# Nico59000/Ternary-image-codec

Measured on AMD Instinct MI355X. Metric: Mpix/s encode+decode 8K RS(26,20), higher is better.
Workload: dtype u8

## Files before the change

### ternary-image-codec_amd/csrc/t3_api.cpp

```cpp
#include <hip/hip_runtime.h>
#include <math.h>
#include <stdio.h>
#include <stdlib.h>
#include <string.h>

#include <algorithm>
#include <atomic>
#include <map>
#include <mutex>
#include <string>
#include <system_error>
#include <thread>
#include <tuple>
#include <vector>

#include "../../include/t3hip.h"
#include "t3_ctx.hpp"
#include "t3_host.hpp"
#include "t3_kernels.h"
#include "t3_decode.h"

using namespace t3;

namespace {
// ... 252 lines not shown
      fprintf(stderr, "[t3 stamps]   CUs seen=%zu  CUs holding n WGs: 1:%d 2:%d 3:%d 4:%d 5:%d 6+:%d\n", per_cu.size(), hist[1], hist[2], hist[3], hist[4], hist[5], hist[6] + hist[7]);
      fprintf(stderr, "[t3 stamps]   mean WG lifetime (us) per XCC:"); for (int x = 0; x < 8; ++x) fprintf(stderr, " %d:%.1f(n=%d)", x, xn[x] ? xl[x] / xn[x] : 0.0, xn[x]); fprintf(stderr, "\n");
      double ln[8] = {0}; int cn[8] = {0}; for (auto& kv : per_cu) { const size_t n = std::min<size_t>(kv.second.size(), 7); for (uint32_t v : kv.second) { ln[n] += v * 0.01; ++cn[n]; } }
      fprintf(stderr, "[t3 stamps]   mean WG lifetime (us) by WGs on its CU:"); for (int n = 1; n < 8; ++n) if (cn[n]) fprintf(stderr, " %d:%.1f", n, ln[n] / cn[n]); fprintf(stderr, "\n");
      fprintf(stderr, "[t3 stamps]   hw_id samples: %08x %08x %08x %08x\n", (unsigned)h16[8], (unsigned)h16[16 + 8], (unsigned)h16[32 + 8], (unsigned)h16[16 * 100 + 8]); }
    double acc[8] = {0, 0, 0, 0, 0, 0, 0, 0};
    for (uint32_t w = 0; w < grid; ++w) for (int i = 0; i < 8; ++i) acc[i] += (double)h[8 * w + i];
    fprintf(stderr, "[t3 stamps] grid=%u tiles=%u  mean cycles/WG: stage=%.0f p1=%.0f p2=%.0f p3=%.0f total=%.0f  clock=%.3f GHz\n", grid, e.a.n_tiles,
            acc[0] / grid, acc[1] / grid, acc[2] / grid, acc[3] / grid, acc[4] / grid, acc[4] / acc[5] * 0.1);
    { uint64_t s0 = ~0ull, s1 = 0, e0 = ~0ull, e1 = 0; for (uint32_t w = 0; w < grid; ++w) { const uint64_t st = h[8 * w + 3], en = st + h[8 * w + 5]; s0 = std::min(s0, st); s1 = std::max(s1, st); e0 = std::min(e0, en); e1 = std::max(e1, en); }
      int late = 0; for (uint32_t w = 0; w < grid; ++w) if (h[8 * w + 3] - s0 > 1000) ++late;
      fprintf(stderr, "[t3 stamps]   timeline (us from first start): last start=%.2f first end=%.2f last end=%.2f  WGs starting >10us late=%d\n", (s1 - s0) * 0.01, (e0 - s0) * 0.01, (e1 - s0) * 0.01, late);
      fprintf(stderr, "[t3 stamps]   lds_bytes=%u block=%u\n", e.a.lds_bytes, e.block); }
    fprintf(stderr, "[t3 stamps]   p1 split (wave 0): prefetch issue=%.0f convert=%.0f barrier wait=%.0f\n", acc[6] / grid, acc[7] / grid, acc[1] / grid);
    { double il = 0; for (uint32_t w = 0; w < grid; ++w) il += (double)h16[16 * w + 10]; fprintf(stderr, "[t3 stamps]   2-D permutation pass (in p2): %.0f\n", il / grid); }
    return T3_OK;
}
#endif

int launch_enc(Ctx& c, EncLaunch& e, hipStream_t s) {
    uint32_t grid; { const int rc = resident_grid(c, e.fn, (int)e.block, e.a.lds_bytes, e.a.n_tiles, true, &grid); if (rc) return rc; }
#ifdef T3_STAMPS
    static uint64_t* d_dbg = nullptr; static int calls = 0;
    if (!d_dbg) HIPCHK(hipMalloc((void**)&d_dbg, 16 * 8 * 4096));
    HIPCHK(hipMemsetAsync(d_dbg, 0, 16 * 8 * 4096, s));
    e.a.dbg = d_dbg;
#endif
    tile_tickets_held(c, s, 0, grid, &e.a.tile_ctr, &e.a.n_classes);
    void* args[] = {(void*)&e.a};
    HIPCHK(hipLaunchKernel(e.fn, dim3(grid), dim3(e.block), args, e.a.lds_bytes, s));
// ... 360 lines not shown
    t3_layout L; int rc = plan(n_raw, *cfg, L); if (rc) return rc;
    *n_out = L.out_words; if (L.out_words > cap) return T3_E_CAPACITY;
    std::lock_guard<std::recursive_mutex> hl(c.host_mu);
    void *di, *dout;
    { std::lock_guard<std::mutex> lk(c.mu); rc = scratch_held(c, Scratch::HostIn, n_units * (fe == FE_PIXELS ? 6 : 9) + 64, &di); if (rc) return rc; rc = scratch_held(c, Scratch::HostOut, L.out_words * 9 + 64, &dout); if (rc) return rc; }
    rc = encode_host_pipelined(c, fe, in, n_units, cfg, out, L, di, dout);
    if (rc != 1) return rc;
    if (n_units) HIPCHK(hipMemcpyAsync(di, in, n_units * (fe == FE_PIXELS ? 6 : 9), hipMemcpyHostToDevice, c.stream));
    rc = encode_dev(fe, di, n_units, cfg, dout, L.out_words, n_out, c.stream); if (rc) return rc;
    if (L.out_words) HIPCHK(hipMemcpyAsync(out, dout, L.out_words * 9, hipMemcpyDeviceToHost, c.stream));
    HIPCHK(hipStreamSynchronize(c.stream)); return T3_OK;
}
int t3hip_encode_profile(const void* raw, uint64_t n_raw, const t3_cfg* cfg, void* out, uint64_t cap, uint64_t* n_out) { return encode_host(FE_WORDS, raw, n_raw, cfg, out, cap, n_out); }
int t3hip_encode_frame(const void* px, uint64_t n_px, const t3_cfg* cfg, void* out, uint64_t cap, uint64_t* n_out) { return encode_host(FE_PIXELS, px, n_px, cfg, out, cap, n_out); }

int t3hip_event_create(void** ev) { if (!ctx().ready) return T3_E_NODEVICE; hipEvent_t e; HIPCHK(hipEventCreate(&e)); *ev = e; return T3_OK; }
int t3hip_event_record(void* ev, void* stream) { HIPCHK(hipEventRecord((hipEvent_t)ev, (hipStream_t)stream)); return T3_OK; }
int t3hip_event_elapsed_ms(void* a, void* b, float* ms) { HIPCHK(hipEventSynchronize((hipEvent_t)b)); HIPCHK(hipEventElapsedTime(ms, (hipEvent_t)a, (hipEvent_t)b)); return T3_OK; }
int t3hip_event_destroy(void* ev) { HIPCHK(hipEventDestroy((hipEvent_t)ev)); return T3_OK; }

}

namespace t3 {
int encode_rgb_fused(const void* d_rgb, uint64_t n_px, const t3_cfg* cfg, void* d_out, uint64_t cap, uint64_t* n_out, hipStream_t s) { return encode_dev(FE_RGB, d_rgb, n_px, cfg, d_out, cap, n_out, s); }
int scratch(Ctx& c, Scratch kind, size_t bytes, void** out, hipStream_t s) { std::lock_guard<std::mutex> lk(c.mu); return scratch_held(c, kind, bytes, out, s); }
void tile_tickets(Ctx& c, hipStream_t s, int kind, uint32_t grid, uint32_t** ctr, uint32_t* n_classes) { std::lock_guard<std::mutex> lk(c.mu); tile_tickets_held(c, s, kind, grid, ctr, n_classes); }
int resident_grid(Ctx& c, const void* fn, int threads, uint32_t lds_bytes, uint64_t n_items, bool round_lds_units, uint32_t* grid) {
    static std::map<std::tuple<const void*, int, int, uint32_t>, int> occ; static std::mutex occ_mu;
    int per_cu;
    {
        std::lock_guard<std::mutex> lk(occ_mu);
// ... 70 lines not shown
```

### ternary-image-codec_amd/csrc/t3_api_decode.cpp

```cpp
#include <hip/hip_runtime.h>
#include <math.h>
#include <stdio.h>
#include <string.h>

#include <stdlib.h>

#include <algorithm>
#include <mutex>
#include <vector>

#include "../../include/t3hip.h"
#include "t3_ctx.hpp"
#include "t3_decode.h"
#include "t3_host.hpp"
#include "t3_window.h"

using namespace t3;

namespace {
struct HdrCheck { HdrExpect ex; uint32_t hs; uint32_t* verdict; const uint8_t* in; };

int launch_hdr_compare(const HdrCheck* h, hipStream_t s) {
    if (!h) return T3_OK;
    hipLaunchKernelGGL(hdr_compare_kernel, dim3(1), dim3(128), 0, s, h->in, h->ex, h->hs, h->verdict);
// ... 152 lines not shown
    void* args[] = {(void*)&a};
    HIPCHK(hipLaunchKernel(p.fn, dim3(grid), dim3(p.threads), args, a.lds_bytes, s));
#ifdef T3_DEC_STAMPS
    if (++calls == 8 && p.tickets) {
        std::vector<uint64_t> h(16 * grid);
        HIPCHK(hipStreamSynchronize(s));
        HIPCHK(hipMemcpy(h.data(), d_dbg, h.size() * 8, hipMemcpyDeviceToHost));
        double acc[16] = {0};
        for (uint32_t w = 0; w < grid; ++w) for (int i = 0; i < 16; ++i) acc[i] += (double)h[16 * w + i];
        fprintf(stderr, "[t3 dec stamps] grid=%u (%d per CU) tiles=%u lds=%u  mean cycles/WG: producer sets+e1=%.0f barrier=%.0f total=%.0f | consumer bm=%.0f rendezvous=%.0f d5=%.0f barrier=%.0f total=%.0f  clock=%.3f GHz  us/WG=%.1f\n",
                grid, (int)((grid + c.n_cu - 1) / c.n_cu), a.n_tiles, a.lds_bytes, acc[0] / grid, acc[1] / grid, acc[6] / grid, acc[8 + 2] / grid, acc[8 + 3] / grid, acc[8 + 4] / grid, acc[8 + 5] / grid, acc[8 + 6] / grid,
                acc[6] / acc[7] * 0.1, acc[7] / grid * 0.01);
        uint64_t s0 = ~0ull, s1 = 0, e1 = 0; int late = 0;
        for (uint32_t w = 0; w < grid; ++w) { s0 = std::min(s0, h[16 * w + 2]); s1 = std::max(s1, h[16 * w + 2]); e1 = std::max(e1, h[16 * w + 3]); }
        for (uint32_t w = 0; w < grid; ++w) if (h[16 * w + 2] - s0 > 1000) ++late;
        fprintf(stderr, "[t3 dec stamps]   timeline (us from first loop start): last start=%.1f last end=%.1f  workgroups starting >10 us late=%d\n", (s1 - s0) * 0.01, (e1 - s0) * 0.01, late);
    }
#endif
    return T3_OK;
}

struct UepPlan { DecUepArgs a; const void* fn; uint32_t grid; };
int plan_fixed_uep(uint64_t body_bytes, uint32_t hdr_syms, const t3_cfg& cfg, const t3_layout& L, const ScrCycle& sc,
                   void* d_out, uint64_t units, uint32_t* d_fail, UepPlan& p) {
    if (L.n_raw_words == 0 || L.n_sym + (1u << 20) >= (1ull << 32) || body_bytes + hdr_syms >= (1ull << 32)) return 1;
    if (getenv("T3HIP_TWO_KERNEL_DECODE") != nullptr) return 1;
    if (body_bytes >= (1ull << 28)) return 1;
    const bool il = L.interleave2d != 0 && cfg.tile_w > 1;
    DecUepArgs& a = p.a; memset(&a, 0, sizeof a);
    int gk[kUepMaxGrp]; uint32_t gn[kUepMaxGrp];
// ... 462 lines not shown
```

### ternary-image-codec_amd/csrc/t3_api_record.cpp

```cpp
#include <hip/hip_runtime.h>
#include <stdlib.h>
#include <string.h>

#include <algorithm>
#include <mutex>
#include <vector>

#include "../../include/t3hip.h"
#include "t3_crc.h"
#include "t3_ctx.hpp"

using namespace t3;

namespace {
struct CrcOp {
    uint32_t col[32];
    uint32_t apply(uint32_t v) const { uint32_t r = 0; for (int b = 0; b < 32; ++b) if (v >> b & 1u) r ^= col[b]; return r; }
    static CrcOp compose(const CrcOp& a, const CrcOp& b) { CrcOp r; for (int i = 0; i < 32; ++i) r.col[i] = a.apply(b.col[i]); return r; }
    static CrcOp identity() { CrcOp r; for (int b = 0; b < 32; ++b) r.col[b] = 1u << b; return r; }
    static CrcOp zero_byte() {
        CrcOp r;
        for (int b = 0; b < 32; ++b) { uint32_t v = 1u << b; for (int i = 0; i < 8; ++i) v = (v & 1u) ? (0xEDB88320u ^ (v >> 1)) : (v >> 1); r.col[b] = v; }
        return r;
    }
// ... 51 lines not shown
    if (mfma) {
        CrcMArgs& m = p.m;
        m.data = d_data; m.n_bytes = n_bytes; m.n_rounds = (uint32_t)(n_bytes >> 11);
        const uint32_t slots = crc_slots(c);
        m.rounds_per_wave = (uint32_t)std::max<uint64_t>(8, ((uint64_t)m.n_rounds + slots - 1) / slots);
        m.afrag = c.crc.afrag4; m.zpow = c.crc.zpow; m.chunk_crc = acc; m.sym_sum = acc + 1;
        m.tail_len = (uint32_t)(n_bytes - ((uint64_t)m.n_rounds << 11));
        const uint32_t tail_wg = m.tail_len ? 1u : 0u;
        if (knob.blocked) {
            const uint64_t waves = ((uint64_t)m.n_rounds + m.rounds_per_wave - 1) / m.rounds_per_wave;
            p.form = CrcForm::Fp4Blocked; p.m_grid = (uint32_t)((waves + 3) / 4 + tail_wg);
        } else {
            int l = 0;
            while (l + 1 < kCrcStrideLevels && (uint64_t)crc_stride_w(slots, l) * 8 > m.n_rounds) ++l;
            m.stride_waves = crc_stride_w(slots, l); m.afb = c.crc.afb + (size_t)l * 64 * 4;
            p.form = CrcForm::Fp4Strided; p.m_grid = m.stride_waves / 4 + tail_wg;
            if (partials && !knob.atomics && p.m_grid <= std::min(cap_wg, kRecordPartialWgs)) { m.partials = partials; p.n_partials = p.m_grid; }
        }
    } else {
        p.form = CrcForm::Tables;
        CrcArgs& t = p.t;
        t.data = d_data; t.n_bytes = n_bytes; t.chunk_bytes = 2304;
        t.n_chunks = (uint32_t)((n_bytes + t.chunk_bytes - 1) / t.chunk_bytes);
        t.chunk_crc = acc; t.sym_sum = acc + 1; t.zpow = c.crc.zpow;
        p.t_grid = (t.n_chunks + 255) / 256;
    }
    p.zero_acc = p.n_partials == 0;
    return p;
}

// ... 24 lines not shown
    int rc = upload(tab.zpow, z); if (rc) return rc;
    HIPCHK(hipMalloc((void**)&tab.acc, 64));
    std::vector<uint32_t> a4((size_t)14 * 64 * 4, 0u);
    static const uint32_t recip[4] = {4u, 2u, 1u, 1u};
    CrcOp to_end[65]; to_end[0] = CrcOp::identity();
    for (int n = 1; n <= 64; ++n) to_end[n] = CrcOp::compose(CrcOp::zero_byte(), to_end[n - 1]);
    for (int st = 0; st < 8; ++st) for (int kh = 0; kh < 2; ++kh) for (int pos = 0; pos < 32; ++pos) {
        const int j = pos >> 3, bit = 4 * (pos & 7) + j, o = 32 * kh + 4 * st + (bit >> 3);
        const uint32_t vec = to_end[64 - o].apply(1u << (bit & 7));
        for (int m = 0; m < 32; ++m) if (vec >> m & 1u) a4[((size_t)st * 64 + m + 32 * kh) * 4 + j] |= recip[j] << (4 * (pos & 7));
    }
    for (int st = 8; st < 14; ++st) remainder_slice(CrcOp::append_zero_bytes(st == 8 ? 2048u : 64u << (st - 9)), &a4[(size_t)st * 64 * 4]);
    rc = upload(tab.afrag4, a4); if (rc) return rc;
    std::vector<uint32_t> fb((size_t)kCrcStrideLevels * 64 * 4, 0u);
    for (int l = 0; l < kCrcStrideLevels; ++l) remainder_slice(CrcOp::append_zero_bytes(2048ull * crc_stride_w(crc_slots(c), l)), &fb[(size_t)l * 64 * 4]);
    return upload(tab.afb, fb);
}
}

extern "C" {

uint64_t t3hip_frame_record_scratch_bytes(uint64_t) { return 64 + 8ull * kRecordPartialWgs; }
int t3hip_frame_record_dev(const void* d_words, uint64_t n_words, uint64_t frame_idx, const t3_cfg* cfg, t3_frame_record* d_rec,
                           void* d_scratch, uint64_t scratch_bytes, void* stream) {
    Ctx& c = ctx(); if (!c.ready) return T3_E_NODEVICE;
    if (!cfg || !d_rec || (n_words && !d_words) || !d_scratch || scratch_bytes < 8) return T3_E_ARG;
    hipStream_t s = (hipStream_t)stream;
    const uint64_t n_bytes = 9 * n_words;
    uint32_t* parts = scratch_bytes >= 64 + 8 ? (uint32_t*)((uint8_t*)d_scratch + 64) : nullptr;
    const uint32_t cap_wg = parts ? (uint32_t)std::min<uint64_t>((scratch_bytes - 64) / 8, kRecordPartialWgs) : 0u;
    const CrcPlan p = plan_crc(c, (const uint8_t*)d_words, n_bytes, (uint32_t*)d_scratch, parts, cap_wg);
// ... 30 lines not shown
```

### ternary-image-codec_amd/csrc/t3_crc.h

```cpp
#pragma once
#include <stdint.h>

namespace t3 {

constexpr int kCrcPows = 40;
struct CrcArgs {
    const uint8_t* data; uint64_t n_bytes; uint32_t chunk_bytes; uint32_t n_chunks;
    uint32_t* chunk_crc; uint32_t* sym_sum;
    const uint32_t* zpow;
};

struct CrcMArgs {
    const uint8_t* data; uint64_t n_bytes;
    uint32_t n_rounds, rounds_per_wave;
    uint32_t stride_waves;
    const uint32_t* afb;
    const uint32_t* afrag;
    const uint32_t* zpow;
    uint32_t* chunk_crc; uint32_t* sym_sum;
    uint32_t* partials;
    uint32_t tail_len;
};
constexpr uint32_t kRecordPartialWgs = 1024;

#if defined(__HIPCC__)
__global__ void crc_chunks_kernel(const CrcArgs a);
__global__ void crc_fp4_kernel(const CrcMArgs a);
__global__ void frame_record_kernel(const uint32_t* acc, uint32_t lead, const uint8_t* words, uint64_t n_words, uint64_t frame_idx, uint32_t profile, uint32_t mode, void* rec, const uint32_t* partials, uint32_t n_partials);
#endif

}
```

### ternary-image-codec_amd/csrc/t3_crc_fp4.hip

```cpp
#include <hip/hip_runtime.h>
#include <stdint.h>

#include "../../include/t3hip.h"
#include "t3_crc.h"

#ifndef T3_CRC_DEPTH
#define T3_CRC_DEPTH 4
#endif
#ifndef T3_CRC_NT
#define T3_CRC_NT 0
#endif

namespace t3 {

typedef int v8i_ __attribute__((ext_vector_type(8)));
typedef float v16f_ __attribute__((ext_vector_type(16)));

namespace {
typedef float v2f_ __attribute__((ext_vector_type(2)));
__device__ __forceinline__ uint4 ld16(const uint8_t* q) {
#if T3_CRC_NT
    typedef uint32_t u4_ __attribute__((ext_vector_type(4)));
    const u4_ v = __builtin_nontemporal_load((const u4_*)q); return make_uint4(v[0], v[1], v[2], v[3]);
#else
    return *(const uint4*)q;
#endif
}
__device__ __forceinline__ uint32_t wave_apply4(const uint32_t* __restrict__ op, uint32_t x, uint32_t lane) {
    uint32_t v = (lane < 32u && ((x >> lane) & 1u)) ? op[lane] : 0u;
#pragma unroll
    for (int o = 32; o > 0; o >>= 1) v ^= __shfl_xor(v, o);
    return v;
}
__device__ __forceinline__ v16f_ mfma4(const uint32_t (&A)[4], const uint32_t b0, const uint32_t b1, const uint32_t b2, const uint32_t b3, const v16f_ acc) {
    const v8i_ a = {(int)A[0], (int)A[1], (int)A[2], (int)A[3], 0, 0, 0, 0}, b = {(int)b0, (int)b1, (int)b2, (int)b3, 0, 0, 0, 0};
    return __builtin_amdgcn_mfma_scale_f32_32x32x64_f8f6f4(a, b, acc, 4, 4, 0, 0x7F7F7F7F, 0, 0x7F7F7F7F);
}
__device__ __forceinline__ void parity_nibbles(const v16f_& acc, uint32_t (&f)[4]) {
    const v2f_ m01 = {8388608.0f, 524288.0f}, m23 = {32768.0f, 2048.0f};
#pragma unroll
    for (int g = 0; g < 4; ++g) {
        const v2f_ lo = v2f_{acc[4 * g], acc[4 * g + 1]} + m01, hi = v2f_{acc[4 * g + 2], acc[4 * g + 3]} + m23;
        f[g] = (__float_as_uint(lo[0]) & 0x1u) | (__float_as_uint(lo[1]) & 0x10u) | (__float_as_uint(hi[0]) & 0x100u) | (__float_as_uint(hi[1]) & 0x1000u);
    }
}
__device__ __forceinline__ v16f_ mfma_round(const uint32_t (&A)[9][4], const uint32_t (&w)[8], v16f_ acc) {
#pragma unroll
    for (int s = 0; s < 8; ++s) acc = mfma4(A[s], w[s] & 0x11111111u, w[s] & 0x22222222u, w[s] & 0x44444444u, (w[s] >> 1) & 0x44444444u, acc);
    return acc;
}
}

__global__ __launch_bounds__(256) void crc_fp4_kernel(const CrcMArgs a) {
    __shared__ uint32_t red[2 * 16];
    __shared__ uint32_t zp[kCrcPows * 32];
    for (uint32_t e = threadIdx.x; e < (uint32_t)kCrcPows * 32u; e += blockDim.x) zp[e] = a.zpow[e];
    __syncthreads();
    const uint32_t lane = threadIdx.x & 63u, n = lane & 31u, kh = lane >> 5, wave = __builtin_amdgcn_readfirstlane(threadIdx.x >> 6);
    const uint32_t tail_wg = a.tail_len ? 1u : 0u;
    const bool in_tail_wg = blockIdx.x < tail_wg;
    const uint32_t wave_g = (blockIdx.x - tail_wg) * (blockDim.x >> 6) + wave;
    const uint32_t W = a.stride_waves;
    uint64_t r0, r1, step;
    if (in_tail_wg) { r0 = r1 = 0; step = 1; }
    else if (W) { r0 = wave_g; r1 = a.n_rounds; step = W; }
    else { r0 = min((uint64_t)wave_g * a.rounds_per_wave, (uint64_t)a.n_rounds); r1 = min(r0 + a.rounds_per_wave, (uint64_t)a.n_rounds); step = 1; }
    uint32_t A[9][4];
#pragma unroll
    for (int s = 0; s < 9; ++s) {
        const uint4 q = (s == 8 && W) ? *(const uint4*)(a.afb + (size_t)lane * 4u) : *(const uint4*)(a.afrag + ((size_t)s * 64u + lane) * 4u);
        A[s][0] = q.x; A[s][1] = q.y; A[s][2] = q.z; A[s][3] = q.w;
    }
    const uint64_t pstep = 2048u * step;
    const uint8_t* p = a.data + r0 * 2048u + 64u * n + 32u * kh;
    const v16f_ zero = {0, 0, 0, 0, 0, 0, 0, 0, 0, 0, 0, 0, 0, 0, 0, 0};
    uint32_t f[4] = {0, 0, 0, 0}, sum = 0;
    constexpr uint32_t kDepth = T3_CRC_DEPTH;
    uint4 Q[kDepth][2];
    uint64_t r_end = r0;
#pragma unroll
    for (uint32_t d = 0; d < kDepth; ++d) { Q[d][0] = make_uint4(0, 0, 0, 0); Q[d][1] = Q[d][0]; if (r0 + d * step < r1) { Q[d][0] = ld16(p + pstep * d); Q[d][1] = ld16(p + pstep * d + 16); } }
    for (uint64_t r = r0; r < r1; r += kDepth * step, p += pstep * kDepth) {
#pragma unroll
        for (uint32_t d = 0; d < kDepth; ++d) {
            if (r + d * step >= r1) break;
            r_end = r + d * step + 1u;
            const uint32_t w[8] = {Q[d][0].x, Q[d][0].y, Q[d][0].z, Q[d][0].w, Q[d][1].x, Q[d][1].y, Q[d][1].z, Q[d][1].w};
            if (r + (d + kDepth) * step < r1) { Q[d][0] = ld16(p + pstep * (d + kDepth)); Q[d][1] = ld16(p + pstep * (d + kDepth) + 16); }
#pragma unroll
            for (int i = 0; i < 8; ++i) sum = __builtin_amdgcn_sad_u8(w[i], 0u, sum);
            parity_nibbles(mfma_round(A, w, mfma4(A[8], f[0], f[1], f[2], f[3], zero)), f);
        }
    }
    if (in_tail_wg && wave == 0) {
        const uint8_t* t = a.data + ((uint64_t)a.n_rounds << 11);
        const int32_t lo = (int32_t)(64u * n + 32u * kh + a.tail_len) - 2048;
        uint32_t w[8] = {0, 0, 0, 0, 0, 0, 0, 0};
        if (lo > -32) {
            uint32_t b[32];
#pragma unroll
            for (int32_t i = 0; i < 32; ++i) b[i] = t[max(lo + i, 0)];
#pragma unroll
            for (int32_t i = 0; i < 32; ++i) w[i >> 2] |= (lo + i >= 0 ? b[i] : 0u) << (8 * (i & 3));
        }
#pragma unroll
        for (int i = 0; i < 8; ++i) sum = __builtin_amdgcn_sad_u8(w[i], 0u, sum);
        parity_nibbles(mfma_round(A, w, zero), f);
    }
#pragma unroll
    for (int b = 0; b < 5; ++b) {
        const uint4 q = *(const uint4*)(a.afrag + ((size_t)(9 + b) * 64u + lane) * 4u);
        const uint32_t Ab[4] = {q.x, q.y, q.z, q.w};
        uint32_t m[4]; parity_nibbles(mfma4(Ab, f[0], f[1], f[2], f[3], zero), m);
        if (((31u - n) >> b) & 1u) { f[0] = m[0]; f[1] = m[1]; f[2] = m[2]; f[3] = m[3]; }
    }
#pragma unroll
    for (int o = 16; o > 0; o >>= 1) {
#pragma unroll
        for (int g = 0; g < 4; ++g) f[g] ^= __shfl_xor(f[g], o);
    }
    uint32_t part = 0;
#pragma unroll
    for (uint32_t e = 0; e < 16; ++e) part |= ((f[e >> 2] >> (4u * (e & 3u))) & 1u) << ((e & 3u) + 8u * (e >> 2) + 4u * kh);
    part |= __shfl_xor(part, 32);
#pragma unroll
    for (int o = 32; o > 0; o >>= 1) sum += __shfl_xor(sum, o);
    uint64_t rest = in_tail_wg ? 0u : W ? (r_end > r0 ? a.n_bytes - r_end * 2048u : 0u) : a.n_bytes - r1 * 2048u;
    for (int j = 0; rest; ++j, rest >>= 1) if (rest & 1u) part = wave_apply4(zp + 32 * j, part, lane);
    if (lane == 0) { red[2 * wave] = part; red[2 * wave + 1] = sum; }
    __syncthreads();
    if (threadIdx.x == 0) {
        uint32_t x = 0, t = 0;
        for (uint32_t w = 0; w < (blockDim.x >> 6); ++w) { x ^= red[2 * w]; t += red[2 * w + 1]; }
        if (a.partials) { a.partials[2u * blockIdx.x] = x; a.partials[2u * blockIdx.x + 1u] = t; }
        else { if (x) atomicXor(a.chunk_crc, x); if (t) atomicAdd(a.sym_sum, t); }
    }
}

}
```

### ternary-image-codec_amd/csrc/t3_ctx.hpp

```cpp
#pragma once
#include <hip/hip_runtime.h>
#include <stdint.h>

#include <algorithm>
#include <functional>
#include <map>
#include <mutex>
#include <string>
#include <utility>
#include <vector>

#include "../../include/t3hip.h"
#include "t3_device.h"
#include "t3_host.hpp"

namespace t3 {

struct RsTables; struct FxTables; struct QuantTables;

template <class T> void free_dev(T*& p) { if (p) (void)hipFree((void*)p); p = nullptr; }
template <class T> void free_pinned(T*& p) { if (p) (void)hipHostFree((void*)p); p = nullptr; }

struct LutImage { uint32_t* d_img = nullptr; uint32_t bytes = 0; uint32_t k_off[4] = {0, 0, 0, 0}; uint32_t* d_afrag = nullptr; };

// ... 3 lines not shown
    uint32_t* synd_T = nullptr; uint32_t* synd_T16 = nullptr;
    uint8_t* fx2_small = nullptr;
    uint32_t* synd_lut[4] = {}; uint32_t synd_lut_bytes[4] = {};
    uint32_t* roots[4] = {};
    uint32_t* synd_afrag[4] = {};
    void release() {
        free_dev(fxtab); free_dev(fma); free_dev(synd_T); free_dev(synd_T16); free_dev(fx2_small);
        for (int i = 0; i < 4; ++i) { free_dev(synd_lut[i]); synd_lut_bytes[i] = 0; free_dev(roots[i]); free_dev(synd_afrag[i]); }
    }
};
struct CrcTables {
    uint32_t* zpow = nullptr;
    uint32_t* acc = nullptr;
    uint32_t* afrag4 = nullptr;
    uint32_t* afb = nullptr;
    std::mutex acc_mu;
    void release() { free_dev(zpow); free_dev(acc); free_dev(afrag4); free_dev(afb); }
};
struct RgbTables {
    QuantTables* quant = nullptr;
    uint8_t* chroma_q = nullptr;
    uint8_t* dequant = nullptr;
    void release() { free_dev(quant); free_dev(chroma_q); free_dev(dequant); }
};
struct Mailboxes {
    uint8_t* header = nullptr;
    uint32_t* fail = nullptr; uint32_t* d_fail = nullptr;
    void release() { free_pinned(header); free_pinned(fail); d_fail = nullptr; }
};

enum class Scratch {
    HostIn, HostOut,
// ... 80 lines not shown
```

### ternary-image-codec_amd/csrc/t3_decode_fused.hip

```cpp
#include <hip/hip_runtime.h>
#include <stdint.h>

#include "../../include/t3hip.h"
#include "t3_decode.h"
#include "t3_decode_fx.h"
#include "t3_decode_fx2.h"

namespace t3 {

namespace {
__device__ __forceinline__ void barrier_lds2() { asm volatile("s_waitcnt lgkmcnt(0)\n\ts_barrier" ::: "memory"); }
typedef uint32_t v4u32 __attribute__((ext_vector_type(4)));
struct __attribute__((packed, aligned(2))) V4a2 { v4u32 v; };
__device__ __forceinline__ v4u32 load16(const uint8_t* p) { return __builtin_nontemporal_load(&((const V4a2*)p)->v); }

template <bool BCN> struct Run { v4u32 w; };
template <> struct Run<true> { v4u32 w; uint32_t w4, x; };
template <bool BCN>
__device__ __forceinline__ Run<BCN> load_run(const DecFx2Args& a, const uint8_t* body, const uint32_t g0) {
    Run<BCN> r;
    if constexpr (!BCN) r.w = load16(body + g0);
    else {
        uint32_t nb0 = 0, c = a.bcn_slot - g0;
        if (g0 >= a.bcn_slot) { const uint32_t u = g0 - a.bcn_slot, j = __umulhi(u, a.bcn_div.mul) >> a.bcn_div.sh; nb0 = j + 1u; c = a.bcn_pb - (u - j * a.bcn_pb); }
// ... 93 lines not shown

#ifndef T3_DEC_WAVES_PER_EU
#define T3_DEC_WAVES_PER_EU 6
#endif
#ifdef T3_DEC_STAMPS
#define T3D_STAMP(i) do { const uint64_t t_ = __builtin_amdgcn_s_memtime(); st_acc[i] += t_ - st_prev; st_prev = t_; } while (0)
#else
#define T3D_STAMP(i) do { } while (0)
#endif

template <int R, bool RGB, bool BCN>
__global__ __launch_bounds__(T3_DEC_PX_THREADS, T3_DEC_WAVES_PER_EU) void decode_fixed_px_kernel(const DecFx2Args a) {
    constexpr uint32_t TCOP = T3_DEC_PX_TCOP, TBASE = kFx2TPx, MT = kFx2ModPx, QCAP = kFx2QCap;
    constexpr uint32_t NW = T3_DEC_PX_THREADS / 128;
    const uint32_t tid = threadIdx.x, lane = tid & 63u, wave = __builtin_amdgcn_readfirstlane(tid >> 6);
    const uint32_t grid = gridDim.x;
    const bool dyn = a.tile_ctr != nullptr;
    const uint32_t NC = dyn ? a.n_classes : 1u, cls = blockIdx.x % NC;
    const uint32_t wgc = (grid - cls + NC - 1u) / NC;
    uint32_t* const ctr = a.tile_ctr + 64u * cls;
    auto draw = [&]() -> uint32_t { return cls + NC * (wgc + atomicAdd(ctr, 1u)); };
    if (tid == 0) *(uint32_t*)(lds + kFx2Next + 4u) = dyn ? draw() : blockIdx.x + grid;
    uint32_t* const failp = a.verdict ? (uint32_t*)(lds + kFx2FailWg) : a.fail;
    if (tid == 0) *(uint32_t*)(lds + kFx2FailWg) = 0u;
    stage_tables<TCOP, TBASE, MT>(a, tid, blockDim.x);
    if constexpr (RGB) { if (tid < 82u) *(uint32_t*)(lds + a.dq_off + 4u * tid) = ((const uint32_t*)a.dq)[tid]; }
    __syncthreads();
#ifdef T3_DEC_STAMPS
    uint64_t st_acc[6] = {0, 0, 0, 0, 0, 0}, st_prev = __builtin_amdgcn_s_memtime(), st_t0 = st_prev, st_rt0 = __builtin_amdgcn_s_memrealtime();
#endif
// ... 22 lines not shown
        for (uint32_t p = 0; p < 2; ++p) for (uint32_t q = 0; q < 2; ++q) geo[p][q] = fx2_geo<R>(wave * 128u + p * 64u + q * 32u + n, n_items, a.nb, a.div_nb, 0u, off0[p][q]);
        auto has = [&](uint32_t pass, uint32_t set, uint32_t tile) -> bool { Geo g = geo[pass][set]; asm volatile("" : "+v"(g)); return fx2_has_block<R>(g, tile, a.n_tiles, a.nb); };
        auto run_of = [&](uint32_t pass, uint32_t set, uint32_t tile) -> Run<BCN> { return load_run<BCN>(a, body, has(pass, set, tile) ? off0[pass][set] + tile * t_off + 10u * h : 0u); };
        Run<BCN> PA, PB;
        PA.w = v4u32{0, 0, 0, 0}; PB.w = PA.w; if constexpr (BCN) { PA.x = 16u << 8; PB.x = PA.x; PA.w4 = 0; PB.w4 = 0; }
        if (cur < a.n_tiles) { PA = run_of(0, 0, cur); PB = run_of(0, 1, cur); }
        for (uint32_t k = 0; cur < a.n_tiles; ++k) {
            const uint32_t tile = cur, buf = k & 1u;
            const uint32_t y_off = a.y_off + buf * a.y_stride, q_off = a.q_off + buf * a.q_stride;
            const uint32_t u2 = 2u * mod3u(tile * a.nb), toff = tile * t_off;
            uint32_t raw; asm volatile("" : "=v"(raw));
#pragma unroll
            for (uint32_t pass = 0; pass < 2; ++pass) {
                uint32_t LA[4], LB[4];
                run_bytes<BCN>(PA, LA); run_bytes<BCN>(PB, LB);
                if (pass == 1u) {
                    asm volatile("" : "+v"(LA[0]), "+v"(LA[1]), "+v"(LA[2]), "+v"(LA[3]), "+v"(LB[0]), "+v"(LB[1]), "+v"(LB[2]), "+v"(LB[3]));
                    if (tid == 0u && dyn) raw = atomicAdd(ctr, 1u);
                }
                {
                    const uint32_t np = pass ^ 1u, nt = pass == 0 ? tile : nxt;
                    if (nt < a.n_tiles) { PA = run_of(np, 0, nt); PB = run_of(np, 1, nt); }
                }
                if (wave * 128u + pass * 64u < n_items) {
                    Geo gA = geo[pass][0], gB = geo[pass][1]; asm volatile("" : "+v"(gA), "+v"(gB));
                    const Blk bA = fx2_block(gA, off0[pass][0] + toff, fx2_has_block<R>(gA, tile, a.n_tiles, a.nb), u2, y_off);
                    const Blk bB = fx2_block(gB, off0[pass][1] + toff, fx2_has_block<R>(gB, tile, a.n_tiles, a.nb), u2, y_off);
                    const Synd sA = fx2_set<R, TCOP, TBASE, MT>(bA, LA, lane, a.af_off, a.pat_off);
                    Synd sB; sB.lo = 0; sB.hi = 0;
                    if (wave * 128u + pass * 64u + 32u < n_items) sB = fx2_set<R, TCOP, TBASE, MT>(bB, LB, lane, a.af_off, a.pat_off);
// ... 44 lines not shown
        }
    }
    if (dyn && tid == 0u) {
        if (a.verdict) { const uint32_t wgf = *(const uint32_t*)(lds + kFx2FailWg); if (wgf) atomicAdd(a.fail, wgf); }
        asm volatile("s_waitcnt vmcnt(0)" ::: "memory");
        if (atomicAdd(a.tile_ctr + 64u * NC, 1u) == grid - 1u) {
            if (a.verdict) a.verdict[1] = atomicExch(a.fail, 0u);
            for (uint32_t c = 0; c <= NC; ++c) __hip_atomic_store(a.tile_ctr + 64u * c, 0u, __ATOMIC_RELAXED, __HIP_MEMORY_SCOPE_AGENT);
        }
    }
#ifdef T3_DEC_STAMPS
    if ((tid == 0 || tid == 64u * NW) && a.dbg) {
        uint64_t* d = a.dbg + 16ull * blockIdx.x + (tid ? 8 : 0);
        for (int i = 0; i < 6; ++i) d[i] = st_acc[i];
        d[6] = __builtin_amdgcn_s_memtime() - st_t0; d[7] = __builtin_amdgcn_s_memrealtime() - st_rt0;
        if (tid == 0) { d[2] = st_rt0; d[3] = __builtin_amdgcn_s_memrealtime(); }
    }
#endif
}

template <int R, bool BCN>
__global__ __launch_bounds__(512, T3_DEC_WAVES_PER_EU) void decode_fixed_kernel(const DecFx2Args a) {
    constexpr uint32_t TCOP = 32, TBASE = kFx2TSeq, MT = kFx2ModSeq;
    const uint32_t tid = threadIdx.x, nthr = blockDim.x, lane = tid & 63u, wave = __builtin_amdgcn_readfirstlane(tid >> 6);
    stage_tables<TCOP, TBASE, MT>(a, tid, nthr);
    __syncthreads();
    const uint8_t* body = a.in + a.hdr_syms;
    const uint32_t n_items = 9u * a.nb;
    const uint32_t units_tile = (a.TS / 26u) * 3u;
    const uint32_t n = lane & 31u, h = lane >> 5;
    uint32_t offA, offB;
// ... 48 lines not shown
```

### ternary-image-codec_amd/csrc/t3_kernels.hip

```cpp
#include <hip/hip_runtime.h>
#include <stdint.h>
#include <type_traits>

#include "t3_device.h"
#include "t3_rs_core.h"

namespace t3 {

extern __shared__ __attribute__((aligned(16))) uint8_t lds[];
#define T3_LDS_PTR(T, a) ((const __attribute__((address_space(3))) T*)(uintptr_t)(a))
#define T3_LDS_WPTR(T, a) ((__attribute__((address_space(3))) T*)(uintptr_t)(a))
typedef uint32_t u32x2 __attribute__((ext_vector_type(2)));
typedef uint32_t u32x4 __attribute__((ext_vector_type(4)));
typedef uint32_t u32x2a4 __attribute__((ext_vector_type(2), aligned(4)));
__device__ __forceinline__ uint32_t lds_u8(uint32_t a)  { return *T3_LDS_PTR(uint8_t, a); }
__device__ __forceinline__ uint32_t lds_u32(uint32_t a) { return *T3_LDS_PTR(uint32_t, a); }

__device__ __forceinline__ uint32_t fdiv(uint32_t n, const DevDiv& d) { return d.d <= 1 ? n : (__umulhi(n, d.mul) >> d.sh); }
__device__ __forceinline__ uint32_t fdiv2(uint32_t n, const DevDiv& d) { return __umulhi(n, d.mul) >> d.sh; }

__device__ __forceinline__ uint32_t div3(uint32_t x)  { return __umul24(x, 171u) >> 9; }
__device__ __forceinline__ uint32_t div9(uint32_t x)  { return __umul24(x, 228u) >> 11; }
__device__ __forceinline__ uint32_t div27(uint32_t x) { return __umul24(x, 152u) >> 12; }
__device__ __forceinline__ uint32_t div81(uint32_t x) { return __umul24(x, 405u) >> 15; }
// ... 866 lines not shown
        case 3: asm volatile("s_waitcnt vmcnt(3) lgkmcnt(0)\n\ts_barrier" ::: "memory"); break;
        case 4: asm volatile("s_waitcnt vmcnt(4) lgkmcnt(0)\n\ts_barrier" ::: "memory"); break;
        case 7: asm volatile("s_waitcnt vmcnt(7) lgkmcnt(0)\n\ts_barrier" ::: "memory"); break;
        case 8: asm volatile("s_waitcnt vmcnt(8) lgkmcnt(0)\n\ts_barrier" ::: "memory"); break;
        default: barrier_all(); break;
    }
}

template <int FE, int IL, int RSEL, bool BCN>
__device__ __forceinline__ void encode_body(const EncArgs& a) {
    constexpr uint32_t GS = fe_px(FE) ? kGroupSyms : kGroupSymsW;
    constexpr uint32_t GBf = FE == FE_PIXELS ? kGroupBytes : FE == FE_RGB ? kGroupBytesRgb : kGroupBytesW;
    constexpr int SH = RSEL != 0 ? 2 : 3;
    const uint32_t tid = threadIdx.x, nthr = blockDim.x, lane = tid & 63u, wave = __builtin_amdgcn_readfirstlane(tid >> 6), nwv = nthr >> 6;
    const uint32_t TS = 9u * a.Lq;

    if (tid == 0) {
#pragma unroll
        for (int b = 0; b < 9; ++b) {
            BandRow r; r.k = a.band_k[b]; r.nbt = a.band_nb_tile[b]; r.blocks = a.band_blocks[b]; r.lut_off = a.band_lut_off[b];
            r.pad_ = 0; r.boff6 = a.band_boff6[b]; r.body_off = a.band_body_off[b];
            *(BandRow*)(lds + 32 * b) = r;
        }
#pragma unroll
        for (int b = 0; b < 10; ++b) *(uint32_t*)(lds + 288 + 4 * b) = a.band_first[b];
#pragma unroll
        for (int i = 0; i < 12; ++i) *(uint32_t*)(lds + 336 + 4 * i) = a.scr[i];
        if constexpr (RSEL == 1) {
#pragma unroll
            for (int gi = 0; gi < kMaxGrp; ++gi) {
// ... 73 lines not shown
    const uint32_t wgc = (gridDim.x - cls + NC - 1u) / NC;
    const uint32_t w0 = fe_px(FE) ? min(a.p1_wpp, nwv - 1u) : min(2u * min(a.p1_wpp, nwv / 2u), nwv - 1u);
    const bool excl = dyn && w0 + 1u < nwv;
    const uint32_t n_pf = nwv - w0 - (excl ? 1u : 0u);
    uint32_t par = 0, rot = 0;
    for (uint32_t tile = blockIdx.x, nxt = dyn ? cls + NC * (wgc + blockIdx.x / NC) : blockIdx.x + gridDim.x, nn = 0; tile < a.n_tiles;
         tile = nxt, nxt = nn, par ^= 1u, rot = (rot + w0 >= nwv ? rot + w0 - nwv : rot + w0)) {
        const uint32_t vw = fast ? (wave >= rot ? wave - rot : wave + nwv - rot) : wave;
        const bool drawer = dyn && lane == 0u && vw == nwv - 1u;
        const uint32_t S0 = tile * TS;
        const uint32_t stage = a.stage_off + (fast ? par * a.stage_stride : 0u);
        uint32_t symb = a.sym_off;
        if constexpr (fast) {
            barrier_input(younger);
            T3_STAMP(0);
            if (drawer) *(uint32_t*)(lds + 328) = cls + NC * (2u * wgc + atomicAdd(ctr, 1u));
#ifndef T3_ABL_NO_PREFETCH
            if (nxt < a.n_tiles && vw >= w0 && vw - w0 < n_pf) stage_tile(tile_in(nxt * TS), a.stage_off + (par ^ 1u) * a.stage_stride, vw - w0, n_pf);
#endif
            T3_STAMP(4);
            uint32_t u_lo = S0, u_hi = S0 + TS;
            bool placed = false;
#ifndef T3_ABL_NO_P1
            if constexpr (fe_px(FE)) {
                const TileIn T = tile_in(S0);
                u_hi = T.hi[0];
                P1Run r0 = p1_run<FE>(T.lo[0], T.hi[0], stage + T.off[0]), r1 = p1_run<FE>(T.lo[1], T.hi[1], stage + T.off[1]), r2 = p1_run<FE>(T.lo[2], T.hi[2], stage + T.off[2]);
                if (T.n < 1u) r0.n_units = 0; if (T.n < 2u) r1.n_units = 0; if (T.n < 3u) r2.n_units = 0;
                u_lo = T.lo[0];
                if constexpr (IL == 2) {
// ... 184 lines not shown
            (void)did;
        }
#endif
        T3_STAMP(2);
    }
    if (dyn && lane == 0u && wave == nwv - 1u) {
        asm volatile("s_waitcnt vmcnt(0)" ::: "memory");
        if (atomicAdd(a.tile_ctr + 64u * NC, 1u) == gridDim.x - 1u) {
            for (uint32_t c = 0; c <= NC; ++c) __hip_atomic_store(a.tile_ctr + 64u * c, 0u, __ATOMIC_RELAXED, __HIP_MEMORY_SCOPE_AGENT);
        }
    }
#ifdef T3_STAMPS
    if (tid == 0 && a.dbg) {
        uint64_t* d = a.dbg + 16ull * blockIdx.x;
        d[8] = __builtin_amdgcn_s_getreg(31 << 11 | 4); d[9] = __builtin_amdgcn_s_getreg(31 << 11 | 20);
        d[0] = st_acc[0]; d[1] = st_acc[1]; d[2] = st_acc[2] + st_acc[3]; d[3] = st_rt0; d[10] = st_acc[3];
        d[4] = __builtin_amdgcn_s_memtime() - st_t0; d[5] = __builtin_amdgcn_s_memrealtime() - st_rt0; d[6] = st_acc[4]; d[7] = st_acc[5];
    }
#endif
}

#ifndef T3_ENC_WAVES_PER_EU
#define T3_ENC_WAVES_PER_EU 6
#endif
template <int FE, int IL, int RSEL, bool BCN>
__global__ __launch_bounds__(512, T3_ENC_WAVES_PER_EU) void encode_kernel_k(const EncArgs a) { encode_body<FE, IL, RSEL, BCN>(a); }
template <int FE, int IL, bool BCN>
__global__ __launch_bounds__(512, T3_ENC_WAVES_PER_EU) void encode_kernel_uep(const EncArgs a) { encode_body<FE, IL, 1, BCN>(a); }
template <int FE, int IL>
__global__ __launch_bounds__(1024) void encode_kernel_mixed(const EncArgs a) { encode_body<FE, IL, 0, false>(a); }

// ... 77 lines not shown
```

Before: 122,300.

## Precompute CRC distance tables, use DPP reductions, disable event system fence

```diff
diff --git a/ternary-image-codec_amd/csrc/t3_api.cpp b/ternary-image-codec_amd/csrc/t3_api.cpp
--- a/ternary-image-codec_amd/csrc/t3_api.cpp
+++ b/ternary-image-codec_amd/csrc/t3_api.cpp
@@ -290,6 +290,7 @@
       fprintf(stderr, "[t3 stamps]   lds_bytes=%u block=%u\n", e.a.lds_bytes, e.block); }
     fprintf(stderr, "[t3 stamps]   p1 split (wave 0): prefetch issue=%.0f convert=%.0f barrier wait=%.0f\n", acc[6] / grid, acc[7] / grid, acc[1] / grid);
     { double il = 0; for (uint32_t w = 0; w < grid; ++w) il += (double)h16[16 * w + 10]; fprintf(stderr, "[t3 stamps]   2-D permutation pass (in p2): %.0f\n", il / grid); }
+    { double pr = 0; for (uint32_t w = 0; w < grid; ++w) pr += (double)h16[16 * w + 11]; fprintf(stderr, "[t3 stamps]   prologue (kernel entry -> first tile's input landed, wave 0): mean %.0f cycles/WG\n", pr / grid); }
     return T3_OK;
 }
 #endif
@@ -680,7 +681,10 @@
 int t3hip_encode_profile(const void* raw, uint64_t n_raw, const t3_cfg* cfg, void* out, uint64_t cap, uint64_t* n_out) { return encode_host(FE_WORDS, raw, n_raw, cfg, out, cap, n_out); }
 int t3hip_encode_frame(const void* px, uint64_t n_px, const t3_cfg* cfg, void* out, uint64_t cap, uint64_t* n_out) { return encode_host(FE_PIXELS, px, n_px, cfg, out, cap, n_out); }
 
-int t3hip_event_create(void** ev) { if (!ctx().ready) return T3_E_NODEVICE; hipEvent_t e; HIPCHK(hipEventCreate(&e)); *ev = e; return T3_OK; }
+#ifndef T3_EVENT_FLAGS
+#define T3_EVENT_FLAGS hipEventDisableSystemFence
+#endif
+int t3hip_event_create(void** ev) { if (!ctx().ready) return T3_E_NODEVICE; hipEvent_t e; HIPCHK(hipEventCreateWithFlags(&e, T3_EVENT_FLAGS)); *ev = e; return T3_OK; }
 int t3hip_event_record(void* ev, void* stream) { HIPCHK(hipEventRecord((hipEvent_t)ev, (hipStream_t)stream)); return T3_OK; }
 int t3hip_event_elapsed_ms(void* a, void* b, float* ms) { HIPCHK(hipEventSynchronize((hipEvent_t)b)); HIPCHK(hipEventElapsedTime(ms, (hipEvent_t)a, (hipEvent_t)b)); return T3_OK; }
 int t3hip_event_destroy(void* ev) { HIPCHK(hipEventDestroy((hipEvent_t)ev)); return T3_OK; }
diff --git a/ternary-image-codec_amd/csrc/t3_api_decode.cpp b/ternary-image-codec_amd/csrc/t3_api_decode.cpp
--- a/ternary-image-codec_amd/csrc/t3_api_decode.cpp
+++ b/ternary-image-codec_amd/csrc/t3_api_decode.cpp
@@ -190,6 +190,7 @@
         uint64_t s0 = ~0ull, s1 = 0, e1 = 0; int late = 0;
         for (uint32_t w = 0; w < grid; ++w) { s0 = std::min(s0, h[16 * w + 2]); s1 = std::max(s1, h[16 * w + 2]); e1 = std::max(e1, h[16 * w + 3]); }
         for (uint32_t w = 0; w < grid; ++w) if (h[16 * w + 2] - s0 > 1000) ++late;
+        fprintf(stderr, "[t3 dec stamps]   prologue (kernel entry -> first tile's input landed, wave 0): mean %.0f cycles/WG\n", acc[4] / grid);
         fprintf(stderr, "[t3 dec stamps]   timeline (us from first loop start): last start=%.1f last end=%.1f  workgroups starting >10 us late=%d\n", (s1 - s0) * 0.01, (e1 - s0) * 0.01, late);
     }
 #endif
diff --git a/ternary-image-codec_amd/csrc/t3_api_record.cpp b/ternary-image-codec_amd/csrc/t3_api_record.cpp
--- a/ternary-image-codec_amd/csrc/t3_api_record.cpp
+++ b/ternary-image-codec_amd/csrc/t3_api_record.cpp
@@ -89,6 +89,7 @@
             int l = 0;
             while (l + 1 < kCrcStrideLevels && (uint64_t)crc_stride_w(slots, l) * 8 > m.n_rounds) ++l;
             m.stride_waves = crc_stride_w(slots, l); m.afb = c.crc.afb + (size_t)l * 64 * 4;
+            m.dist_lo = c.crc.dist_lo; m.dist_hi = c.crc.dist_hi; m.last_mod = (m.n_rounds - 1u) % m.stride_waves;
             p.form = CrcForm::Fp4Strided; p.m_grid = m.stride_waves / 4 + tail_wg;
             if (partials && !knob.atomics && p.m_grid <= std::min(cap_wg, kRecordPartialWgs)) { m.partials = partials; p.n_partials = p.m_grid; }
         }
@@ -143,7 +144,16 @@
     rc = upload(tab.afrag4, a4); if (rc) return rc;
     std::vector<uint32_t> fb((size_t)kCrcStrideLevels * 64 * 4, 0u);
     for (int l = 0; l < kCrcStrideLevels; ++l) remainder_slice(CrcOp::append_zero_bytes(2048ull * crc_stride_w(crc_slots(c), l)), &fb[(size_t)l * 64 * 4]);
-    return upload(tab.afb, fb);
+    rc = upload(tab.afb, fb); if (rc) return rc;
+    const uint32_t w0 = crc_stride_w(crc_slots(c), 0);
+    std::vector<uint32_t> lo((size_t)2048 * 32), hi(((size_t)w0 + 1) * 32);
+    const CrcOp one = CrcOp::zero_byte(), round = CrcOp::append_zero_bytes(2048);
+    CrcOp op = CrcOp::identity();
+    for (uint32_t n = 0; n < 2048; ++n, op = CrcOp::compose(one, op)) memcpy(&lo[(size_t)n * 32], op.col, sizeof op.col);
+    op = CrcOp::identity();
+    for (uint32_t n = 0; n <= w0; ++n, op = CrcOp::compose(round, op)) memcpy(&hi[(size_t)n * 32], op.col, sizeof op.col);
+    rc = upload(tab.dist_lo, lo); if (rc) return rc;
+    return upload(tab.dist_hi, hi);
 }
 }
 
diff --git a/ternary-image-codec_amd/csrc/t3_crc.h b/ternary-image-codec_amd/csrc/t3_crc.h
--- a/ternary-image-codec_amd/csrc/t3_crc.h
+++ b/ternary-image-codec_amd/csrc/t3_crc.h
@@ -17,6 +17,9 @@
     const uint32_t* afb;
     const uint32_t* afrag;
     const uint32_t* zpow;
+    const uint32_t* dist_lo;
+    const uint32_t* dist_hi;
+    uint32_t last_mod;
     uint32_t* chunk_crc; uint32_t* sym_sum;
     uint32_t* partials;
     uint32_t tail_len;
diff --git a/ternary-image-codec_amd/csrc/t3_crc_fp4.hip b/ternary-image-codec_amd/csrc/t3_crc_fp4.hip
--- a/ternary-image-codec_amd/csrc/t3_crc_fp4.hip
+++ b/ternary-image-codec_amd/csrc/t3_crc_fp4.hip
@@ -26,11 +26,24 @@
     return *(const uint4*)q;
 #endif
 }
+template <int kCtrl> __device__ __forceinline__ uint32_t dpp_(uint32_t v) { return (uint32_t)__builtin_amdgcn_update_dpp(0, (int)v, kCtrl, 0xF, 0xF, true); }
+__device__ __forceinline__ uint32_t rows_(uint32_t v, bool add) {
+    const uint32_t r0 = __builtin_amdgcn_readlane((int)v, 0), r1 = __builtin_amdgcn_readlane((int)v, 16), r2 = __builtin_amdgcn_readlane((int)v, 32), r3 = __builtin_amdgcn_readlane((int)v, 48);
+    return add ? r0 + r1 + r2 + r3 : r0 ^ r1 ^ r2 ^ r3;
+}
+__device__ __forceinline__ uint32_t wave_xor(uint32_t v) {
+    v ^= dpp_<0xB1>(v); v ^= dpp_<0x4E>(v); v ^= dpp_<0x141>(v); v ^= dpp_<0x140>(v);
+    return rows_(v, false);
+}
+__device__ __forceinline__ uint32_t wave_sum(uint32_t v) {
+    v += dpp_<0xB1>(v); v += dpp_<0x4E>(v); v += dpp_<0x141>(v); v += dpp_<0x140>(v);
+    return rows_(v, true);
+}
+__device__ __forceinline__ uint32_t wave_apply_col(uint32_t col, uint32_t x, uint32_t lane) {
+    return wave_xor((lane < 32u && ((x >> lane) & 1u)) ? col : 0u);
+}
 __device__ __forceinline__ uint32_t wave_apply4(const uint32_t* __restrict__ op, uint32_t x, uint32_t lane) {
-    uint32_t v = (lane < 32u && ((x >> lane) & 1u)) ? op[lane] : 0u;
-#pragma unroll
-    for (int o = 32; o > 0; o >>= 1) v ^= __shfl_xor(v, o);
-    return v;
+    return wave_apply_col(lane < 32u ? op[lane] : 0u, x, lane);
 }
 __device__ __forceinline__ v16f_ mfma4(const uint32_t (&A)[4], const uint32_t b0, const uint32_t b1, const uint32_t b2, const uint32_t b3, const v16f_ acc) {
     const v8i_ a = {(int)A[0], (int)A[1], (int)A[2], (int)A[3], 0, 0, 0, 0}, b = {(int)b0, (int)b1, (int)b2, (int)b3, 0, 0, 0, 0};
@@ -53,9 +66,6 @@
 
 __global__ __launch_bounds__(256) void crc_fp4_kernel(const CrcMArgs a) {
     __shared__ uint32_t red[2 * 16];
-    __shared__ uint32_t zp[kCrcPows * 32];
-    for (uint32_t e = threadIdx.x; e < (uint32_t)kCrcPows * 32u; e += blockDim.x) zp[e] = a.zpow[e];
-    __syncthreads();
     const uint32_t lane = threadIdx.x & 63u, n = lane & 31u, kh = lane >> 5, wave = __builtin_amdgcn_readfirstlane(threadIdx.x >> 6);
     const uint32_t tail_wg = a.tail_len ? 1u : 0u;
     const bool in_tail_wg = blockIdx.x < tail_wg;
@@ -65,26 +75,32 @@
     if (in_tail_wg) { r0 = r1 = 0; step = 1; }
     else if (W) { r0 = wave_g; r1 = a.n_rounds; step = W; }
     else { r0 = min((uint64_t)wave_g * a.rounds_per_wave, (uint64_t)a.n_rounds); r1 = min(r0 + a.rounds_per_wave, (uint64_t)a.n_rounds); step = 1; }
+    const uint64_t pstep = 2048u * step;
+    const uint8_t* p = a.data + r0 * 2048u + 64u * n + 32u * kh;
+    const v16f_ zero = {0, 0, 0, 0, 0, 0, 0, 0, 0, 0, 0, 0, 0, 0, 0, 0};
+    uint32_t f[4] = {0, 0, 0, 0}, sum = 0;
+    constexpr uint32_t kDepth = T3_CRC_DEPTH;
+    uint4 Q[kDepth][2];
+#pragma unroll
+    for (uint32_t d = 0; d < kDepth; ++d) { Q[d][0] = make_uint4(0, 0, 0, 0); Q[d][1] = Q[d][0]; if (r0 + d * step < r1) { Q[d][0] = ld16(p + pstep * d); Q[d][1] = ld16(p + pstep * d + 16); } }
+    __builtin_amdgcn_sched_barrier(0);
     uint32_t A[9][4];
 #pragma unroll
     for (int s = 0; s < 9; ++s) {
         const uint4 q = (s == 8 && W) ? *(const uint4*)(a.afb + (size_t)lane * 4u) : *(const uint4*)(a.afrag + ((size_t)s * 64u + lane) * 4u);
         A[s][0] = q.x; A[s][1] = q.y; A[s][2] = q.z; A[s][3] = q.w;
     }
-    const uint64_t pstep = 2048u * step;
-    const uint8_t* p = a.data + r0 * 2048u + 64u * n + 32u * kh;
-    const v16f_ zero = {0, 0, 0, 0, 0, 0, 0, 0, 0, 0, 0, 0, 0, 0, 0, 0};
-    uint32_t f[4] = {0, 0, 0, 0}, sum = 0;
-    constexpr uint32_t kDepth = T3_CRC_DEPTH;
-    uint4 Q[kDepth][2];
-    uint64_t r_end = r0;
-#pragma unroll
-    for (uint32_t d = 0; d < kDepth; ++d) { Q[d][0] = make_uint4(0, 0, 0, 0); Q[d][1] = Q[d][0]; if (r0 + d * step < r1) { Q[d][0] = ld16(p + pstep * d); Q[d][1] = ld16(p + pstep * d + 16); } }
+    uint32_t dcol_lo = 0, dcol_hi = 0;
+    if (W) {
+        const bool moves = !in_tail_wg && wave_g < W && r0 < r1;
+        const uint32_t hi = moves ? (a.last_mod >= wave_g ? a.last_mod - wave_g : a.last_mod + W - wave_g) : 0u;
+        dcol_lo = a.dist_lo[(moves ? a.tail_len : 0u) * 32u + n];
+        dcol_hi = a.dist_hi[hi * 32u + n];
+    }
     for (uint64_t r = r0; r < r1; r += kDepth * step, p += pstep * kDepth) {
 #pragma unroll
         for (uint32_t d = 0; d < kDepth; ++d) {
             if (r + d * step >= r1) break;
-            r_end = r + d * step + 1u;
             const uint32_t w[8] = {Q[d][0].x, Q[d][0].y, Q[d][0].z, Q[d][0].w, Q[d][1].x, Q[d][1].y, Q[d][1].z, Q[d][1].w};
             if (r + (d + kDepth) * step < r1) { Q[d][0] = ld16(p + pstep * (d + kDepth)); Q[d][1] = ld16(p + pstep * (d + kDepth) + 16); }
 #pragma unroll
@@ -114,19 +130,19 @@
         uint32_t m[4]; parity_nibbles(mfma4(Ab, f[0], f[1], f[2], f[3], zero), m);
         if (((31u - n) >> b) & 1u) { f[0] = m[0]; f[1] = m[1]; f[2] = m[2]; f[3] = m[3]; }
     }
-#pragma unroll
-    for (int o = 16; o > 0; o >>= 1) {
-#pragma unroll
-        for (int g = 0; g < 4; ++g) f[g] ^= __shfl_xor(f[g], o);
-    }
     uint32_t part = 0;
 #pragma unroll
     for (uint32_t e = 0; e < 16; ++e) part |= ((f[e >> 2] >> (4u * (e & 3u))) & 1u) << ((e & 3u) + 8u * (e >> 2) + 4u * kh);
-    part |= __shfl_xor(part, 32);
-#pragma unroll
-    for (int o = 32; o > 0; o >>= 1) sum += __shfl_xor(sum, o);
-    uint64_t rest = in_tail_wg ? 0u : W ? (r_end > r0 ? a.n_bytes - r_end * 2048u : 0u) : a.n_bytes - r1 * 2048u;
-    for (int j = 0; rest; ++j, rest >>= 1) if (rest & 1u) part = wave_apply4(zp + 32 * j, part, lane);
+    part = wave_xor(part);
+    sum = wave_sum(sum);
+    if (W) part = wave_apply_col(dcol_hi, wave_apply_col(dcol_lo, part, lane), lane);
+    else {
+        __shared__ uint32_t zp[kCrcPows * 32];
+        for (uint32_t e = threadIdx.x; e < (uint32_t)kCrcPows * 32u; e += blockDim.x) zp[e] = a.zpow[e];
+        __syncthreads();
+        uint64_t rest = in_tail_wg ? 0u : a.n_bytes - r1 * 2048u;
+        for (int j = 0; rest; ++j, rest >>= 1) if (rest & 1u) part = wave_apply4(zp + 32 * j, part, lane);
+    }
     if (lane == 0) { red[2 * wave] = part; red[2 * wave + 1] = sum; }
     __syncthreads();
     if (threadIdx.x == 0) {
diff --git a/ternary-image-codec_amd/csrc/t3_ctx.hpp b/ternary-image-codec_amd/csrc/t3_ctx.hpp
--- a/ternary-image-codec_amd/csrc/t3_ctx.hpp
+++ b/ternary-image-codec_amd/csrc/t3_ctx.hpp
@@ -41,8 +41,10 @@
     uint32_t* acc = nullptr;
     uint32_t* afrag4 = nullptr;
     uint32_t* afb = nullptr;
+    uint32_t* dist_lo = nullptr;
+    uint32_t* dist_hi = nullptr;
     std::mutex acc_mu;
-    void release() { free_dev(zpow); free_dev(acc); free_dev(afrag4); free_dev(afb); }
+    void release() { free_dev(zpow); free_dev(acc); free_dev(afrag4); free_dev(afb); free_dev(dist_lo); free_dev(dist_hi); }
 };
 struct RgbTables {
     QuantTables* quant = nullptr;
diff --git a/ternary-image-codec_amd/csrc/t3_decode_fused.hip b/ternary-image-codec_amd/csrc/t3_decode_fused.hip
--- a/ternary-image-codec_amd/csrc/t3_decode_fused.hip
+++ b/ternary-image-codec_amd/csrc/t3_decode_fused.hip
@@ -131,6 +131,9 @@
     constexpr uint32_t TCOP = T3_DEC_PX_TCOP, TBASE = kFx2TPx, MT = kFx2ModPx, QCAP = kFx2QCap;
     constexpr uint32_t NW = T3_DEC_PX_THREADS / 128;
     const uint32_t tid = threadIdx.x, lane = tid & 63u, wave = __builtin_amdgcn_readfirstlane(tid >> 6);
+#ifdef T3_DEC_STAMPS
+    const uint64_t st_entry = __builtin_amdgcn_s_memtime(); uint64_t st_first = 0;
+#endif
     const uint32_t grid = gridDim.x;
     const bool dyn = a.tile_ctr != nullptr;
     const uint32_t NC = dyn ? a.n_classes : 1u, cls = blockIdx.x % NC;
@@ -183,6 +186,9 @@
             for (uint32_t pass = 0; pass < 2; ++pass) {
                 uint32_t LA[4], LB[4];
                 run_bytes<BCN>(PA, LA); run_bytes<BCN>(PB, LB);
+#ifdef T3_DEC_STAMPS
+                if (k == 0u && pass == 0u) { asm volatile("s_waitcnt vmcnt(0)" ::: "memory"); st_first = __builtin_amdgcn_s_memtime() - st_entry; }
+#endif
                 if (pass == 1u) {
                     asm volatile("" : "+v"(LA[0]), "+v"(LA[1]), "+v"(LA[2]), "+v"(LA[3]), "+v"(LB[0]), "+v"(LB[1]), "+v"(LB[2]), "+v"(LB[3]));
                     if (tid == 0u && dyn) raw = atomicAdd(ctr, 1u);
@@ -257,7 +263,7 @@
         uint64_t* d = a.dbg + 16ull * blockIdx.x + (tid ? 8 : 0);
         for (int i = 0; i < 6; ++i) d[i] = st_acc[i];
         d[6] = __builtin_amdgcn_s_memtime() - st_t0; d[7] = __builtin_amdgcn_s_memrealtime() - st_rt0;
-        if (tid == 0) { d[2] = st_rt0; d[3] = __builtin_amdgcn_s_memrealtime(); }
+        if (tid == 0) { d[2] = st_rt0; d[3] = __builtin_amdgcn_s_memrealtime(); d[4] = st_first; }
     }
 #endif
 }
diff --git a/ternary-image-codec_amd/csrc/t3_kernels.hip b/ternary-image-codec_amd/csrc/t3_kernels.hip
--- a/ternary-image-codec_amd/csrc/t3_kernels.hip
+++ b/ternary-image-codec_amd/csrc/t3_kernels.hip
@@ -904,6 +904,9 @@
     constexpr int SH = RSEL != 0 ? 2 : 3;
     const uint32_t tid = threadIdx.x, nthr = blockDim.x, lane = tid & 63u, wave = __builtin_amdgcn_readfirstlane(tid >> 6), nwv = nthr >> 6;
     const uint32_t TS = 9u * a.Lq;
+#ifdef T3_STAMPS
+    const uint64_t st_entry = __builtin_amdgcn_s_memtime(); uint64_t st_first = 0;
+#endif
 
     if (tid == 0) {
 #pragma unroll
@@ -1007,6 +1010,9 @@
         if constexpr (fast) {
             barrier_input(younger);
             T3_STAMP(0);
+#ifdef T3_STAMPS
+            if (!st_first) st_first = st_prev - st_entry;
+#endif
             if (drawer) *(uint32_t*)(lds + 328) = cls + NC * (2u * wgc + atomicAdd(ctr, 1u));
 #ifndef T3_ABL_NO_PREFETCH
             if (nxt < a.n_tiles && vw >= w0 && vw - w0 < n_pf) stage_tile(tile_in(nxt * TS), a.stage_off + (par ^ 1u) * a.stage_stride, vw - w0, n_pf);
@@ -1221,7 +1227,7 @@
     if (tid == 0 && a.dbg) {
         uint64_t* d = a.dbg + 16ull * blockIdx.x;
         d[8] = __builtin_amdgcn_s_getreg(31 << 11 | 4); d[9] = __builtin_amdgcn_s_getreg(31 << 11 | 20);
-        d[0] = st_acc[0]; d[1] = st_acc[1]; d[2] = st_acc[2] + st_acc[3]; d[3] = st_rt0; d[10] = st_acc[3];
+        d[0] = st_acc[0]; d[1] = st_acc[1]; d[2] = st_acc[2] + st_acc[3]; d[3] = st_rt0; d[10] = st_acc[3]; d[11] = st_first;
         d[4] = __builtin_amdgcn_s_memtime() - st_t0; d[5] = __builtin_amdgcn_s_memrealtime() - st_rt0; d[6] = st_acc[4]; d[7] = st_acc[5];
     }
 #endif
```

After: 126,100, median of 6. 3.1% higher.
